# proycon/analiticcl

Measured on AMD Instinct MI355X. Metric: scored (query,candidate) pairs/sec + queries/sec, 200k-lexicon, len≤16, 1/2/4/8 GPU, higher is better.
Workload: dtype u8

## Files before the change

### analiticcl_amd/csrc/engine.hip

```cpp
#include <hip/hip_runtime.h>

#include <algorithm>
#include <atomic>
#include <functional>
#include <chrono>
#include <cmath>
#include <cstdio>
#include <cstdlib>
#include <cstring>
#include <map>
#include <memory>
#include <mutex>
#include <unordered_map>
#include <numeric>
#include <thread>
#include <type_traits>

#include "engine_internal.h"

namespace anx {

#define HIP_TRY(expr)                                                                          \
  do {                                                                                         \
    hipError_t _e = (expr);                                                                    \
// ... 1008 lines not shown
      if (hipEventElapsedTime(&ms, r.e0, r.e1) == hipSuccess) { auto& a = t.acc[r.name]; a.first += ms; a.second += 1; }
    }
    if (r.e0) (void)hipEventDestroy(r.e0);
    if (r.e1) (void)hipEventDestroy(r.e1);
  }
  t.pending.clear();
  ++t.generation;
}
}
int ktimer_begin(const char* name, hipStream_t st) {
  KTimer& t = ktimer();
  if (!t.on.load(std::memory_order_relaxed)) return -1;
  KTimerRec r;
  r.name = name;
  if (hipEventCreate(&r.e0) != hipSuccess || hipEventCreate(&r.e1) != hipSuccess || hipEventRecord(r.e0, st) != hipSuccess) {
    if (r.e0) (void)hipEventDestroy(r.e0);
    if (r.e1) (void)hipEventDestroy(r.e1);
    return -1;
  }
  std::lock_guard<std::mutex> lk(t.mu);
  if (t.pending.size() >= 0xFFFFu) return -1;
  t.pending.push_back(r);
  return (int)(((t.generation & 0x7FFFu) << 16) | (uint32_t)(t.pending.size() - 1));
}
void ktimer_end(int handle, hipStream_t st) {
  if (handle < 0) return;
  KTimer& t = ktimer();
  std::lock_guard<std::mutex> lk(t.mu);
  const uint32_t idx = (uint32_t)handle & 0xFFFFu;
  if ((((uint32_t)handle >> 16) & 0x7FFFu) != (t.generation & 0x7FFFu) || idx >= t.pending.size()) return;
  KTimerRec& r = t.pending[idx];
  if (hipEventRecord(r.e1, st) == hipSuccess) r.closed = true;
}
void kernel_timer_enable(bool on) {
  KTimer& t = ktimer();
  std::lock_guard<std::mutex> lk(t.mu);
  ktimer_resolve_locked(t);
  t.acc.clear();
  t.on.store(on);
}
bool kernel_timer_read(const char* name, double* total_ms, uint64_t* launches) {
  KTimer& t = ktimer();
  std::lock_guard<std::mutex> lk(t.mu);
  ktimer_resolve_locked(t);
  auto it = t.acc.find(name ? name : "");
  if (it == t.acc.end()) { if (total_ms) *total_ms = 0.0; if (launches) *launches = 0; return false; }
  if (total_ms) *total_ms = it->second.first;
  if (launches) *launches = it->second.second;
  return true;
}

#include "launch_plan.hpp"

template <int NP>
static void launch_scan(ScanArgs A, uint32_t nadj, uint32_t nbits, uint32_t nsad, hipStream_t st, hipEvent_t e0, hipEvent_t e1) {
  (void)hipEventRecord(e0, st);
  const bool gen = A.want_exact || A.qpairs || !A.drop_len;
  if (nadj) {
    A.ntiles = nadj;
    if (gen) hipLaunchKernelGGL((k_scan_adj<true>), dim3((nadj + 3) / 4), dim3(256), 0, st, A);
    else hipLaunchKernelGGL((k_scan_adj<false>), dim3((nadj + 3) / 4), dim3(256), 0, st, A);
    A.tiles += nadj;
    nbits -= nadj;
  }
  if (nbits) {
    A.ntiles = nbits;
    if (A.want_exact || A.qpairs || !A.drop_len) hipLaunchKernelGGL((k_scan_bits<true>), dim3((nbits + 3) / 4), dim3(256), 0, st, A);
    else hipLaunchKernelGGL((k_scan_bits<false>), dim3((nbits + 3) / 4), dim3(256), 0, st, A);
  }
  (void)hipEventRecord(e1, st);
  if (nsad) {
    A.tiles += nbits;
    A.ntiles = nsad;
    hipLaunchKernelGGL((k_scan_sad<NP>), dim3((nsad + 3) / 4), dim3(256), 0, st, A);
  }
}

static int ensure_raw(Batch* b, size_t slots_per_region, std::string& err) {
  uint32_t shift = 10;
  while (((size_t)1 << shift) < slots_per_region) ++shift;
  if (shift > 25) { err = "pair list exceeds 2^31 slots: split the batch"; return ANX_ELIMIT; }
  const size_t cap = (size_t)SCAN_REGIONS << shift;
  if (cap <= b->raw_cap) return ANX_OK;
  for (void* p : {(void*)b->raw, (void*)b->p_score, (void*)b->p_meta})
    if (p) pool_free(p);
  b->raw = nullptr; b->p_score = nullptr; b->p_meta = nullptr; b->raw_cap = 0;
  int rc;
  if ((rc = dalloc(&b->raw, cap, err))) return rc;
  b->raw_cap = cap;
  b->region_shift = shift;
  return ANX_OK;
}
static int ensure_pair_outputs(Batch* b, std::string& err) {
  if (b->p_meta) return ANX_OK;
  int rc;
  if ((rc = dalloc(&b->p_score, b->raw_cap, err)) || (rc = dalloc(&b->p_meta, b->raw_cap, err))) return rc;
  return ANX_OK;
}

static int ensure_surv(Batch* b, size_t cap, std::string& err) {
  if (cap <= b->surv_cap) return ANX_OK;
  for (void* p : {(void*)b->c_rows, (void*)b->r_rows, (void*)b->t_key})
    if (p) pool_free(p);
  b->c_rows = nullptr;
  b->r_rows = nullptr;
  b->t_key = nullptr;
  b->surv_cap = 0;
  int rc;
  if ((rc = dalloc(&b->c_rows, cap, err)) || (rc = dalloc(&b->r_rows, cap, err)) || (rc = dalloc(&b->t_key, cap, err))) return rc;
  b->surv_cap = cap;
  return ANX_OK;
}
static int ensure_surv_records(Batch* b, size_t need, std::string& err) {
  if (need <= b->surv_region_cap) return ANX_OK;
// ... 713 lines not shown
```

### analiticcl_amd/csrc/host_model.cpp

```cpp
#include "host_model.h"
#include "adjacency.h"

#include <sched.h>

#include <thread>

#include <algorithm>
#include <cmath>
#include <cstdio>
#include <cstring>
#include <fstream>
#include <numeric>
#include <sstream>

#include "unicode_tables.inc"

namespace anx {

static std::vector<uint32_t> make_primes() {
  std::vector<uint32_t> p;
  for (uint32_t n = 2; p.size() < 168; ++n) {
    bool prime = true;
    for (uint32_t d : p) {
      if (d * d > n) break;
// ... 448 lines not shown
    for (;;) {
      size_t e = line.find('\t', pos);
      fields.emplace_back(line, pos, e == std::string::npos ? std::string::npos : e - pos);
      if (e == std::string::npos) break;
      pos = e + 1;
    }
    bool havef = false;
    uint32_t freq = 0;
    if (has_freq < 0) {
      if (fields.size() >= 2 && (fields.size() - 2) % 3 == 0) {
        if (parse_u32(fields[1], freq)) { has_freq = 1; havef = true; }
      } else has_freq = 0;
    } else if (has_freq == 1) {
      if (fields.size() < 2 || !parse_u32(fields[1], freq)) {
        err = "Frequency must be an integer (line " + std::to_string(linenr) + ", column 2)";
        return ANX_EINVAL;
      }
      havef = true;
    }
    const uint64_t ref_id = add_to_vocabulary(fields[0].c_str(), havef, freq, p, lexidx);
    const size_t step = has_freq == 1 ? 3 : 2;
    for (size_t i = has_freq == 1 ? 2 : 1; i + step - 1 < fields.size(); i += step) {
      char* endp = nullptr;
      const double score = strtod(fields[i + 1].c_str(), &endp);
      if (fields[i + 1].empty() || *endp) { err = "Variant scores must be a floating point value (line " + std::to_string(linenr) + ")"; return ANX_EINVAL; }
      uint32_t vf = 0;
      if (has_freq == 1 && !parse_u32(fields[i + 2], vf)) { err = "Variant frequency must be an integer (line " + std::to_string(linenr) + ")"; return ANX_EINVAL; }
      add_variant(ref_id, fields[i].c_str(), score, has_freq == 1, vf, transparent ? tp : p, lexidx);
    }
  }
  lexicons.push_back(path);
  return ANX_OK;
}

static int pick_planes(int nsym) {
  const int need = (nsym + 3) / 4;
  for (int v : {8, 16, 24, 32, 42})
    if (need <= v) return v;
  return -1;
}

namespace {
struct SwitchDef { const char* name; void (*set)(Switches&, const char*); };
int flag01(const char* v, int dflt) { return !v ? dflt : (v[0] == '0' ? 0 : 1); }
const SwitchDef kSwitches[] = {
    {"ANX_ENCODE", [](Switches& s, const char* v) { s.encode_host = v && strcmp(v, "host") == 0; }},
    {"ANX_SCAN", [](Switches& s, const char* v) { s.scan_sad = v && strcmp(v, "sad") == 0; }},
    {"ANX_SCAN_WALK", [](Switches& s, const char* v) { s.scan_walk_flat = v && strcmp(v, "flat") == 0; }},
    {"ANX_SCAN_TQ", [](Switches& s, const char* v) { const int x = v ? atoi(v) : 0; s.scan_tq = x >= 1 && x <= 64 ? x : 0; }},
    {"ANX_SCAN_ADJ", [](Switches& s, const char* v) { s.scan_adj = flag01(v, 1); }},
    {"ANX_ADJ_BUILD", [](Switches& s, const char* v) { s.adj_build_host = v && strcmp(v, "host") == 0; }},
    {"ANX_ADJ_CLOSURE", [](Switches& s, const char* v) { const int x = v ? atoi(v) : 2; s.adj_closure = x >= 0 && x <= kAdjMaxClosure ? x : kAdjMaxClosure; }},
    {"ANX_SCAN_CHUNK_FUSED", [](Switches& s, const char* v) { const int x = v ? atoi(v) : 0; s.scan_chunk_fused = x >= 32 && x <= 1024 ? x : 0; }},
    {"ANX_ADJ_FAIL", [](Switches& s, const char* v) { s.adj_fail = flag01(v, 0); }},
    {"ANX_SMALL", [](Switches& s, const char* v) { s.small_path = flag01(v, 1); }},
    {"ANX_SURV_SEG", [](Switches& s, const char* v) { const int x = v ? atoi(v) : 32; s.surv_seg = x >= 0 && x <= 256 ? x : 32; }},
    {"ANX_ENC_PRIORITY", [](Switches& s, const char* v) { s.enc_priority = flag01(v, 1); }},
    {"ANX_HINTS", [](Switches& s, const char* v) { s.hints = flag01(v, 1); }},
    {"ANX_ADJ_MB", [](Switches& s, const char* v) { const long x = v ? atol(v) : 0; s.adj_budget_mb = x > 0 ? x : 16384; }},
    {"ANX_SIG_GROUPS", [](Switches& s, const char* v) { const int x = v ? atoi(v) : 0; s.sig_groups = x >= 1 && x <= 8 ? x : 0; }},
    {"ANX_PREFILTER", [](Switches& s, const char* v) { s.prefilter = flag01(v, 1); }},
    {"ANX_SCORE_FAST", [](Switches& s, const char* v) { s.score_fast = flag01(v, 1); }},
    {"ANX_FS_SPLIT", [](Switches& s, const char* v) { s.fs_split = flag01(v, 1); }},
    {"ANX_FS_PLANES", [](Switches& s, const char* v) { s.fs_planes = flag01(v, 1); }},
    {"ANX_FS_B7", [](Switches& s, const char* v) { s.fs_b7 = flag01(v, 1); }},
    {"ANX_SCAN_FUSE", [](Switches& s, const char* v) { s.fuse_prefilter = flag01(v, 1); }},
    {"ANX_CAP_DIV", [](Switches& s, const char* v) { const long x = v ? atol(v) : 0; s.cap_div = x > 1 ? x : 1; }},
    {"ANX_MAX_BATCH", [](Switches& s, const char* v) { const long x = v ? atol(v) : 0; s.max_batch = x > 0 ? x : (4l << 20); }},
    {"ANX_RUN_OVERLAP", [](Switches& s, const char* v) { s.run_overlap = (v && atoi(v) == 0 && v[0] == '0') ? 0 : 1; }},
    {"ANX_SHARD_POLICY", [](Switches& s, const char* v) { s.shard_by_length = (v && strcmp(v, "range") == 0) ? 0 : 1; }},
    {"ANX_SHARD_MIN", [](Switches& s, const char* v) { const long x = v ? atol(v) : 0; s.shard_min = x > 0 ? x : 8192; }},
    {"ANX_CONFUSABLES", [](Switches& s, const char* v) { s.confusables_host = v && strcmp(v, "host") == 0; }},
    {"ANX_LATTICE", [](Switches& s, const char* v) { s.lattice_host = v && strcmp(v, "host") == 0; }},
    {"ANX_SEARCH_ONEPASS", [](Switches& s, const char* v) { s.search_onepass = flag01(v, 1); }},
    {"ANX_ENCODE_TIMING", [](Switches& s, const char* v) { s.encode_timing = v != nullptr && v[0] != 0 && v[0] != '0'; }},
    {"ANX_SEARCH_TIMING", [](Switches& s, const char* v) { s.search_timing = v != nullptr && v[0] != 0 && v[0] != '0'; }},
    {"ANX_SEARCH_PARTS", [](Switches& s, const char* v) { const int x = v ? atoi(v) : 0; s.search_parts = x >= 1 && x <= 8 ? x : 4; }},
    {"ANX_SEARCH_PART_BYTES", [](Switches& s, const char* v) { const long x = v ? atol(v) : 0; s.search_part_bytes = x > 0 ? x : (4l << 20); }},
    {"ANX_SEARCH_PRIO", [](Switches& s, const char* v) { s.search_prio = flag01(v, 1); }},
    {"ANX_SEARCH_EARLY_OUTPUT", [](Switches& s, const char* v) { s.search_early_output = flag01(v, 1); }},
    {"ANX_SEARCH_FIRST_PCT", [](Switches& s, const char* v) { const int x = v ? atoi(v) : 0; s.search_first_pct = x >= 10 && x <= 100 ? x : 50; }},
    {"ANX_SEARCH_PARTS_MIN", [](Switches& s, const char* v) { const long x = v ? atol(v) : 0; s.search_parts_min = x > 0 ? x : (2l << 20); }},
    {"ANX_LEARN_FOLD", [](Switches& s, const char* v) { s.learn_fold_host = v && strcmp(v, "host") == 0; }},
    {"ANX_LEARN_HASH_BITS", [](Switches& s, const char* v) { const int x = v ? atoi(v) : 63; s.learn_hash_bits = x >= 1 && x <= 63 ? x : 63; }},
};
}
Switches& switches() {
  static Switches sw = []() {
    Switches s;
    for (const SwitchDef& d : kSwitches)
      if (const char* v = getenv(d.name)) d.set(s, v);
    return s;
  }();
  return sw;
}
bool set_switch(const char* name, const char* value) {
  if (!name) return false;
  for (const SwitchDef& d : kSwitches)
    if (strcmp(d.name, name) == 0) { d.set(switches(), value); return true; }
  return false;
}

unsigned usable_hw_threads() {
  static const unsigned cached = []() {
    unsigned n = std::max(1u, std::thread::hardware_concurrency());
    cpu_set_t set;
// ... 256 lines not shown
```

### analiticcl_amd/csrc/host_model.h

```cpp
#pragma once
#include <cstdint>
#include <atomic>
#include <memory>
#include <mutex>
#include <string>
#include <unordered_map>
#include <vector>

#include "../../include/anx.h"
#include "confusables_core.hpp"
#include "contextrules_flat.hpp"

namespace anx {

constexpr int kMaxSymbols = 255;
constexpr int kMaxAlphabet = 166;
constexpr int kMaxAnagramDistance = 12;
constexpr int kMaxEditDistance = 12;

struct AlphabetMember {
  std::string bytes;
  int nchars;
};

struct Alphabet {
  std::vector<std::vector<AlphabetMember>> classes;
  int size() const { return (int)classes.size(); }
  struct Cand { int16_t cls; const AlphabetMember* m; };
  std::vector<Cand> by_first[256];
  int16_t fast[256];
  void index();
  bool scan(const char* text, size_t nbytes, std::vector<int16_t>& out) const;
  int scan_into(const char* text, size_t nbytes, int16_t* out, int cap) const;
};

bool parse_alphabet(const std::string& tsv, Alphabet& out, std::string& err);
struct EncodeTables {
  int16_t fast[256];
  uint32_t coff[257];
  std::vector<uint32_t> cand;
  std::vector<uint8_t> bytes;
  std::vector<uint32_t> lower;
};
void build_encode_tables(const Alphabet& a, EncodeTables& out);
bool first_char_is_lowercase(const char* utf8);
bool is_alphabetic_cp(uint32_t cp);
const uint32_t (*alphabetic_ranges(uint32_t* n))[2];
uint32_t utf8_decode_at(const char* s, size_t avail, int* len);
std::string trim_whitespace(const std::string& s);
unsigned usable_hw_threads();

struct Switches {
  int encode_host = 0;
  int scan_sad = 0;
  int scan_walk_flat = 0;
  int scan_tq = 0;
  int scan_adj = 1;
  int adj_build_host = 0;
  int adj_closure = 2;
  long adj_budget_mb = 16384;
  int sig_groups = 0;
  int prefilter = 1;
  int score_fast = 1;
  int fs_planes = 1;
  int fs_split = 1;
  int fs_b7 = 1;
  int fuse_prefilter = 1;
  long cap_div = 1;
  long max_batch = 4l << 20;
  int run_overlap = 1;
  int shard_by_length = 1;
  long shard_min = 8192;
  int confusables_host = 0;
  int lattice_host = 0;
  int search_onepass = 1;
  int scan_chunk_fused = 0;
  int adj_fail = 0;
  int small_path = 1;
  int enc_priority = 1;
  int hints = 1;
  int encode_timing = 0;
  int search_timing = 0;
  int search_parts = 4;
  long search_parts_min = 2l << 20;
  long search_part_bytes = 4l << 20;
  int search_prio = 1;
  int search_early_output = 1;
  int search_first_pct = 50;
  int surv_seg = 32;
  int learn_fold_host = 0;
  int learn_hash_bits = 63;
};
Switches& switches();
bool set_switch(const char* name, const char* value);

struct VariantRef {
  bool variant_of;
  uint64_t id;
  double score;
};

struct VocabEntry {
  std::string text;
  std::vector<uint8_t> norm;
  uint32_t frequency;
  uint32_t lexindex;
  uint8_t tokencount;
  uint8_t vocabtype;
  bool has_variants = false;
  std::vector<VariantRef> variants;
};

struct BigVal {
  std::vector<uint32_t> w;
  void set_one() { w.assign(1, 1u); }
  void mul_small(uint32_t m);
  int cmp(const BigVal& o) const;
  std::string to_decimal() const;
};

struct LexiconImage {
  int nsym = 0;
  int nplanes = 0;
  uint32_t nclasses = 0, nentries = 0;
  std::vector<uint32_t> cls_planes;
  uint32_t cstride = 0;
  std::vector<uint32_t> cls_bits;
  std::vector<uint8_t> cls_len;
  std::vector<uint32_t> cls_off;
// ... 147 lines not shown
```

### analiticcl_amd/csrc/kernels_scan.hpp

```cpp
#pragma once

enum { RC_RAW = 0, RC_VALID = 1, RC_FUSED = 2 , RC_TESTS = 4 ,
       RC_ADJ = 14 , RC_ADJ_FIRST = 15  };

struct WaveOut {
  uint32_t base, left;
  uint32_t emitted;
  uint32_t nbase;
  uint32_t split;
  uint32_t rbase, rend;
  uint32_t* ctr;
  uint32_t chunk;
};
__device__ inline uint32_t wave_inclusive_scan(uint32_t x) {
  uint32_t v = x;
  v += (uint32_t)__builtin_amdgcn_update_dpp(0, (int)x, 0x111, 0xF, 0xF, false);
  v += (uint32_t)__builtin_amdgcn_update_dpp(0, (int)x, 0x112, 0xF, 0xF, false);
  v += (uint32_t)__builtin_amdgcn_update_dpp(0, (int)x, 0x113, 0xF, 0xF, false);
  v += (uint32_t)__builtin_amdgcn_update_dpp(0, (int)v, 0x114, 0xF, 0xE, false);
  v += (uint32_t)__builtin_amdgcn_update_dpp(0, (int)v, 0x118, 0xF, 0xC, false);
  v += (uint32_t)__builtin_amdgcn_update_dpp(0, (int)v, 0x142, 0xA, 0xF, false);
  v += (uint32_t)__builtin_amdgcn_update_dpp(0, (int)v, 0x143, 0xC, 0xF, false);
  return v;
}
__device__ inline uint32_t wave_reserve(WaveOut& w, uint32_t ntot, uint32_t lane, uint32_t* total_out) {
  const uint32_t incl = wave_inclusive_scan(ntot);
  const uint32_t total = (uint32_t)__builtin_amdgcn_readlane((int)incl, 63);
  *total_out = total;
  w.split = w.left;
  if (total > w.left) {
    const uint32_t rest = total - w.left;
    const uint32_t need = rest > w.chunk ? rest : w.chunk;
    uint32_t b = 0;
    if (lane == 0) b = atomicAdd(&w.ctr[RC_RAW], need);
    w.nbase = w.rbase + __shfl(b, 0);
  }
  return incl - ntot;
}
__device__ inline void wave_reserve_total(WaveOut& w, uint32_t total, uint32_t lane) {
  w.split = w.left;
  if (total > w.left) {
    const uint32_t rest = total - w.left;
    const uint32_t need = rest > w.chunk ? rest : w.chunk;
    uint32_t b = 0;
    if (lane == 0) b = atomicAdd(&w.ctr[RC_RAW], need);
    w.nbase = w.rbase + (uint32_t)__builtin_amdgcn_readfirstlane((int)b);
  }
}
__device__ inline uint32_t wave_slot(const WaveOut& w, uint32_t g) {
  return g < w.split ? w.base + g : w.nbase + (g - w.split);
}
__device__ inline void wave_commit(WaveOut& w, uint32_t total) {
  if (total > w.left) {
    const uint32_t rest = total - w.left;
    const uint32_t need = rest > w.chunk ? rest : w.chunk;
    w.base = w.nbase + rest;
    w.left = need - rest;
  } else {
    w.base += total;
    w.left -= total;
  }
  w.emitted += total;
}
__device__ inline void wave_close(const WaveOut& w, uint32_t lane, uint2* __restrict__ raw) {
  for (uint32_t i = lane; i < w.left; i += 64)
    if (w.base + i < w.rend) raw[w.base + i] = make_uint2(RAW_INVALID, 0u);
  if (lane == 0 && w.emitted) atomicAdd(&w.ctr[RC_VALID], w.emitted);
}

struct ScanArgs {
  const Tile* tiles;
  uint32_t ntiles;
  const uint32_t* q_bits;
  const uint32_t* q_cv;
  const uint32_t* cls_bits;
  const uint32_t* cls_planes;
  const uint4* scan_rec;
  const uint2* scan_rec34;
  uint32_t pad_rec;
  uint32_t cstride;
  uint32_t pad_class;
  const uint8_t* cls_len;
  const uint32_t* cls_off;
  const uint4* sig;
  const uint4* sig_e;
  const uint4* sighash;
  const uint4* sighash_e;
  uint32_t hash_mask;
  const unsigned long long* ball;
  const uint32_t* adj_hdr;
  const uint2* adj_planes;
  const uint32_t* adj_ids;
  const uint32_t* sig_cbeg;
  uint2* raw;
  uint32_t region_cap;
  uint32_t chunk;
  uint32_t chunk_fused;
  uint32_t* rctr;
  const uint32_t* qexact;
  int want_exact;
  int drop_len;
  const uint4* q_rec;
  const uint4* e_rec;
  int fuse;
  uint32_t* qpairs;
  int dbg;
};

__device__ inline int32_t bcnt_acc(uint32_t x, int32_t acc) {
  int32_t r;
  asm("v_bcnt_u32_b32 %0, %1, %2" : "=v"(r) : "v"(x), "v"(acc));
  return r;
}
__device__ inline int32_t bcnt_acc_s(uint32_t x, int32_t acc) {
  int32_t r;
  asm("v_bcnt_u32_b32 %0, %1, %2" : "=v"(r) : "v"(x), "s"(acc));
  return r;
}

template <bool BITS, int NP, bool GEN, bool ADJ = false>
__device__ inline void scan_tile(const ScanArgs& AA, const Tile& t, uint32_t item, uint32_t* __restrict__ stage, uint32_t* __restrict__ hits,
                                 uint32_t* __restrict__ qlds, uint4* __restrict__ qsym, uint32_t* __restrict__ pbuf) {
  ScanArgs A = AA;
  if (!GEN) { A.want_exact = 0; A.qpairs = nullptr; A.drop_len = 1; A.qexact = nullptr; }
  constexpr int CPL = BITS ? 4 : (NP <= 8 ? 4 : NP <= 16 ? 2 : 1);
  constexpr int W = BITS ? NBITPLANES : NP;
  constexpr int QSTRIDE = BITS ? NBITPLANES : NP;
  constexpr uint32_t CHUNK = 64u * CPL;
  const uint32_t lane = threadIdx.x & 63;
  const uint32_t* __restrict__ cls_words = BITS ? A.cls_bits : A.cls_planes;
  const uint8_t* __restrict__ cls_len = A.cls_len;
  const uint32_t* __restrict__ cls_off = A.cls_off;
  uint2* __restrict__ raw = A.raw;
  const uint32_t cstride = A.cstride;
  const uint32_t region = item % SCAN_REGIONS;
  WaveOut wo{0, 0, 0, 0, 0, region * A.region_cap, (region + 1) * A.region_cap, A.rctr + region * RC_STRIDE, A.chunk};
  uint32_t ns = 0;
  uint32_t nchunks = 0;
  uint32_t arend = 0;
  int32_t alc[4] = {0, 0, 0, 0};
  uint2 apl[4] = {};
  uint32_t aid[4] = {};
  auto adj_load = [&](uint32_t row, uint2 (&pl)[4], uint32_t (&id)[4]) {
#pragma unroll
    for (int j = 0; j < 4; ++j) {
      pl[j] = make_uint2(0u, 0u);
      id[j] = A.pad_rec;
      if (row + (uint32_t)j < arend) {
        const size_t p = (size_t)(row + (uint32_t)j) * 64u + lane;
        pl[j] = A.adj_planes[p];
        id[j] = A.adj_ids[p];
      }
    }
  };
  {
    const uint32_t* __restrict__ src = (BITS ? A.q_bits : A.q_cv) + (size_t)t.q0 * QSTRIDE;
    for (uint32_t i = lane; i < t.nq * QSTRIDE; i += 64) qlds[i] = src[i];
  }
  const bool fuse = BITS && A.fuse && t.lq <= 16u && t.d <= 3u;
  if (fuse) wo.chunk = A.chunk_fused;
  if (BITS && fuse && lane < t.nq) qsym[lane] = rec32(A.q_rec, t.q0 + lane)[0];
  constexpr uint32_t PBUF = SCAN_PBUF;
  uint32_t nfused = 0;
  uint32_t npb = 0, phead = 0;

  uint32_t nhits = 0;
  uint32_t counted_only = 0;
  auto emit_dense = [&](bool fin) {
    while (npb >= 64u || (fin && npb)) {
      const uint32_t cnt = npb < 64u ? npb : 64u;
      const bool act = lane < cnt;
      const uint32_t pr = pbuf[(phead + lane) & (PBUF - 1u)];
      const uint32_t e = act ? (pr & 0x3FFFFFFu) : 0u, ql = act ? (pr >> 26) : 0u;
      bool keep = act;
      uint32_t flag = 0u;
      if (ANX_DBG(A.dbg) & 16) keep = false;
      if (BITS && fuse && !(ANX_DBG(A.dbg) & 16)) {
        nfused += cnt;
        const uint4 C = rec32(A.e_rec, e)[0];
        const int lc = (int)(rec32(A.e_rec, e)[1].x & 0xFFu), lq = (int)t.lq, d = (int)t.d;
        const uint4 Q = qsym[ql];
        const bool filt = act && lc <= 16;
        const int ml = lq > lc ? lq : lc;
        constexpr uint32_t M = 0x7F7F7F7Fu;
        bool rej;
        if (__any(filt && ml > 12)) {
          const uint32_t q4[4] = {Q.x & M, Q.y & M, Q.z & M, Q.w & M}, c6[6] = {M, C.x & M, C.y & M, C.z & M, C.w & M, M};
          rej = band_bound_rejects<4, true, true>(q4, c6, filt, d, lq, lc);
        } else if (__any(filt && ml > 8)) {
          const uint32_t q3[3] = {Q.x & M, Q.y & M, Q.z & M}, c5[5] = {M, C.x & M, C.y & M, C.z & M, M};
          rej = band_bound_rejects<3, true, true>(q3, c5, filt, d, lq, lc);
        } else {
          const uint32_t q2[2] = {Q.x & M, Q.y & M}, c4[4] = {M, C.x & M, C.y & M, M};
          rej = band_bound_rejects<2, true, true>(q2, c4, filt, d, lq, lc);
        }
        if (rej) { keep = false; ++counted_only; }
        if (filt) flag = RAW_PREFILTERED;
      }
      if (ANX_DBG(A.dbg) & 32) keep = false;
      const unsigned long long km = __ballot(keep);
      const uint32_t total = (uint32_t)__popcll(km);
      if (total) {
        wave_reserve_total(wo, total, lane);
        if (keep) {
          const uint32_t q = t.q0 + ql;
          uint32_t exact = 0u;
          if (A.want_exact) exact = A.qexact[q] == A.scan_rec[e].w ? 0x80000000u : 0u;
          const uint32_t g = __builtin_amdgcn_mbcnt_hi((uint32_t)(km >> 32), __builtin_amdgcn_mbcnt_lo((uint32_t)km, 0u));
          const uint32_t pos = wave_slot(wo, g);
          if (pos < wo.rend) raw[pos] = make_uint2(q, e | exact | flag);
        }
        wave_commit(wo, total);
      }
      phead = (phead + cnt) & (PBUF - 1u);
      npb -= cnt;
    }
  };
  auto flush = [&]() {
    for (uint32_t r0 = 0; r0 < nhits; r0 += 64) {
      const uint32_t idx = r0 + lane;
      uint32_t c = 0, m = 0, e0 = 0, ne = 0, qb = 0;
      if (idx < nhits) {
        bool count_only;
        if (BITS) {
          const uint32_t hx = reinterpret_cast<const uint16_t*>(hits + SCAN_HITS)[idx];
          m = hits[idx];
          qb = ((hx >> 8) & 1u) << 5;
          count_only = (hx >> 9) & 1u;
          e0 = stage[hx & 0xFFu];
          ne = 1;
          c = A.qpairs ? A.scan_rec[e0].w : 0u;
        } else {
          c = hits[2 * idx];
          m = hits[2 * idx + 1];
          qb = ((c >> 27) & 1u) << 5;
          c &= (1u << 27) - 1u;
          const uint32_t lc = cls_len[c];
          e0 = cls_off[c];
          ne = cls_off[c + 1] - e0;
          const uint32_t diff = lc > t.lq ? lc - t.lq : t.lq - lc;
          count_only = A.drop_len && diff > t.d;
        }
        if (A.qpairs) {
          for (uint32_t mm = m; mm; mm &= mm - 1u) {
            const uint32_t q = t.q0 + qb + (uint32_t)__ffs((int)mm) - 1u;
            if (!A.want_exact || A.qexact[q] == 0xFFFFFFFFu || A.qexact[q] == c) atomicAdd(&A.qpairs[q], ne);
          }
        }
        if (count_only) {
          counted_only += (uint32_t)__popc(m) * ne;
          m = 0;
        }
      }
      if (BITS) {
        while (true) {
          const bool has = m != 0u;
          const unsigned long long bm = __ballot(has);
          if (!bm) break;
          if (has) {
            const uint32_t bit = (uint32_t)__ffs((int)m) - 1u;
            m &= m - 1u;
            pbuf[(phead + npb + __builtin_amdgcn_mbcnt_hi((uint32_t)(bm >> 32), __builtin_amdgcn_mbcnt_lo((uint32_t)bm, 0u))) & (PBUF - 1u)] = e0 | ((qb + bit) << 26);
          }
          npb += (uint32_t)__popcll(bm);
          if (npb >= 64u) emit_dense(false);
// ... 151 lines not shown
      if (!BITS && nhits > SCAN_HITS - CHUNK) flush();
    }
    if (BITS) flush();
  };

  uint32_t* __restrict__ sdelta = stage + CHUNK;
  uint32_t* __restrict__ smask = stage + CHUNK + 64;
  auto stage_runs = [&](bool ok, uint32_t cb, uint32_t n) {
    ok = ok && n != 0u;
    const unsigned long long okm = __ballot(ok);
    if (!okm || (ANX_DBG(A.dbg) & 4)) return;
    const uint32_t cnt = ok ? n : 0u;
    const uint32_t incl = wave_inclusive_scan(cnt);
    const uint32_t carry = ns & 63u;
    const uint32_t total = carry + (uint32_t)__builtin_amdgcn_readlane((int)incl, 63);
    uint32_t wbase = ns - carry;
    const uint32_t endp = carry + incl - 1u;
    if (ok) sdelta[__builtin_amdgcn_mbcnt_hi((uint32_t)(okm >> 32), __builtin_amdgcn_mbcnt_lo((uint32_t)okm, 0u))] = cb + cnt - 1u - endp;
    uint32_t rbase = 0;
    for (uint32_t w0 = 0; w0 < total; w0 += SCAN_MASKW) {
      if (lane < SCAN_MASKW / 32u) smask[lane] = 0u;
      if (ok && endp - w0 < SCAN_MASKW) atomicOr(smask + ((endp - w0) >> 5), 1u << (endp & 31u));
      const uint32_t wend = total < w0 + SCAN_MASKW ? total : w0 + SCAN_MASKW;
      for (uint32_t p0 = w0; p0 < wend; p0 += 64) {
        const uint32_t mlo = (uint32_t)__builtin_amdgcn_readfirstlane((int)smask[((p0 - w0) >> 6) * 2u]), mhi = (uint32_t)__builtin_amdgcn_readfirstlane((int)smask[((p0 - w0) >> 6) * 2u + 1u]);
        const uint32_t r = rbase + __builtin_amdgcn_mbcnt_hi(mhi, __builtin_amdgcn_mbcnt_lo(mlo, 0u));
        rbase += (uint32_t)__popc(mlo) + (uint32_t)__popc(mhi);
        const uint32_t p = p0 + lane;
        const uint32_t id = sdelta[r & 63u] + p;
        if (p >= carry && p < total) stage[wbase + lane] = id;
        if (p0 + 64u <= total) {
          wbase += 64u;
          ns = wbase;
          if (wbase == CHUNK) {
            process();
            ns = 0;
            wbase = 0;
          }
        } else {
          ns = wbase + (total - p0);
        }
      }
    }
  };
  const uint4* __restrict__ sigtab = BITS ? A.sig_e : A.sig;
  if (ADJ) {
    const cptr_u32 hp = (cptr_u32)(A.adj_hdr + (size_t)(t.adj - 1u) * 8u);
    const uint32_t row0 = hp[0], c0 = hp[1], c1 = hp[2], c2 = hp[3], c3 = hp[4], c4 = hp[5], c5 = hp[6], c6 = hp[7];
    uint32_t rbeg = t.k >= 3u ? 0u : t.k == 2u ? c0 : t.k == 1u ? c1 : c2;
    uint32_t rend = t.k >= 3u ? c6 : t.k == 2u ? c5 : t.k == 1u ? c4 : c3;
    if (t.flags & 2u) { rbeg = t.s0; rend = t.s1; }
    arend = row0 + rend;
    if (lane == 0 && rend > rbeg) {
      atomicAdd(&wo.ctr[RC_ADJ], rend - rbeg);
      if (t.flags & 1u) atomicAdd(&wo.ctr[RC_ADJ_FIRST], rend - rbeg);
    }
    uint2 npl[4];
    uint32_t nid[4];
    if (rbeg < rend) adj_load(row0 + rbeg, npl, nid);
    for (uint32_t r = rbeg; r < rend; r += (uint32_t)CPL) {
#pragma unroll
      for (int j = 0; j < 4; ++j) {
        const uint32_t rr = r + (uint32_t)j;
        alc[j] = (int32_t)t.lq - 3 + (int32_t)((rr >= c0) + (rr >= c1) + (rr >= c2) + (rr >= c3) + (rr >= c4) + (rr >= c5));
        apl[j] = npl[j];
        aid[j] = nid[j];
      }
      if (r + (uint32_t)CPL < rend) adj_load(row0 + r + (uint32_t)CPL, npl, nid);
      process();
    }
  } else if (t.balln) {
    const unsigned long long H = 0x8080808080808080ull;
    const unsigned long long sq = (unsigned long long)t.sig_lo | (unsigned long long)t.sig_hi << 32;
    const uint4* __restrict__ htab = BITS ? A.sighash_e : A.sighash;
    for (uint32_t base = 0; base < t.balln; base += 64) {
      const uint32_t i = base + lane;
      bool found = false;
      uint32_t first = 0, count = 0;
      if (i < t.balln) {
        const unsigned long long dl = A.ball[t.ball0 + i];
        const unsigned long long r = ((sq & ~H) + (dl & ~H)) ^ ((sq ^ dl) & H);
        if (!(r & (r << 1) & H)) {
          const uint32_t lo = (uint32_t)r, hi = (uint32_t)(r >> 32);
          uint32_t h = sig_hash(lo, hi) & A.hash_mask;
          for (int p = 0; p < 17; ++p) {
            const uint4 e = htab[h];
            if (!e.w) break;
            if (e.x == lo && e.y == hi) { found = true; first = e.z; count = e.w; break; }
            h = (h + 1u) & A.hash_mask;
          }
        }
      }
      stage_runs(found, first, count);
    }
  } else {
    const uint4* __restrict__ sigp = sigtab + t.s0 + lane;
    uint4 sg_next = t.s0 < t.s1 ? *sigp : make_uint4(0xFFFFFFFFu, 0xFFFFFFFFu, 0u, 0u);
    for (uint32_t sb = t.s0; sb < t.s1; sb += 64) {
      const uint4 sg = sg_next;
      sigp += 64;
      if (sb + 64 < t.s1) sg_next = *sigp;
      const bool ok = __builtin_amdgcn_sad_u8(sg.x, t.sig_lo, __builtin_amdgcn_sad_u8(sg.y, t.sig_hi, 0u)) <= t.k;
      stage_runs(ok, sg.z, sg.w);
    }
  }
  if (!ADJ && ns) process();
  flush();
  if (BITS) emit_dense(true);
  if (A.drop_len) {
    const uint32_t tot = (uint32_t)__builtin_amdgcn_readlane((int)wave_inclusive_scan(counted_only), 63);
    wo.emitted += tot;
  }
  wave_close(wo, lane, raw);
  if (BITS && lane == 0 && nfused) atomicAdd(&wo.ctr[RC_FUSED], nfused);
  if (lane == 0 && nchunks) {
    if (BITS) {
      const uint32_t e[5] = {0u, t.kend & 0xFFu, (t.kend >> 8) & 0xFFu, (t.kend >> 16) & 0xFFu, t.nq};
      for (int k = 1; k <= NBITPLANES; ++k)
        if (e[k] > e[k - 1])
          atomicAdd(reinterpret_cast<unsigned long long*>(wo.ctr + RC_TESTS + 2 * k), (unsigned long long)nchunks * CHUNK * (e[k] - e[k - 1]));
    } else {
      atomicAdd(reinterpret_cast<unsigned long long*>(wo.ctr + RC_TESTS), (unsigned long long)nchunks * CHUNK * t.nq);
    }
  }
}

constexpr uint32_t SCAN_STAGE = 64 * 4 + 64 + SCAN_MASKW / 32;
template <int NP, bool BITS, bool GEN, bool ADJ = false>
__device__ inline void scan_wave(const ScanArgs& A) {
  constexpr int QWORDS = SCAN_TQ * (BITS ? NBITPLANES : NP);
  __shared__ uint32_t s_qlds[4][QWORDS];
  __shared__ __attribute__((aligned(16))) uint32_t s_stage[4][ADJ ? 64 * 4 : SCAN_STAGE];
  __shared__ uint32_t s_hits[4][BITS ? SCAN_HITS + SCAN_HITS / 2 : 2 * SCAN_HITS];
  __shared__ uint4 s_qsym[BITS ? 4 : 1][BITS ? SCAN_TQ : 1];
  __shared__ uint32_t s_pbuf[BITS ? 4 : 1][BITS ? SCAN_PBUF : 1];
  const uint32_t wid = threadIdx.x >> 6;
  const uint32_t item = (uint32_t)__builtin_amdgcn_readfirstlane((int)(blockIdx.x * 4u + wid));
  if (item >= A.ntiles) return;
  const cptr_u32 tp = (cptr_u32)(A.tiles + item);
  Tile t;
  t.q0 = tp[0]; t.nq = tp[1]; t.s0 = tp[2]; t.s1 = tp[3]; t.k = tp[4]; t.lq = tp[5]; t.sig_lo = tp[6]; t.sig_hi = tp[7]; t.kind = tp[8]; t.d = tp[9]; t.kend = tp[10]; t.ball0 = tp[11]; t.balln = tp[12]; t.adj = tp[13]; t.flags = tp[14];
  scan_tile<BITS, NP, GEN, ADJ>(A, t, item, s_stage[wid], s_hits[wid], s_qlds[wid], s_qsym[BITS ? wid : 0], s_pbuf[BITS ? wid : 0]);
}
template <bool GEN>
__global__ __launch_bounds__(256) __attribute__((amdgpu_waves_per_eu(5, 8))) void k_scan_bits(ScanArgs A) { scan_wave<8, true, GEN>(A); }
template <bool GEN>
__global__ __launch_bounds__(256) __attribute__((amdgpu_waves_per_eu(6, 8))) void k_scan_adj(ScanArgs A) { scan_wave<8, true, GEN, true>(A); }
template <int NP>
__global__ __launch_bounds__(256) void k_scan_sad(ScanArgs A) { scan_wave<NP, false, true>(A); }


template <int NP>
__global__ __launch_bounds__(256) void k_scan_small(ScanArgs A) {
  constexpr int QW = NP > NBITPLANES ? NP : NBITPLANES;
  __shared__ uint32_t s_qlds[4][QW];
  __shared__ __attribute__((aligned(16))) uint32_t s_stage[4][SCAN_STAGE];
  __shared__ uint32_t s_hits[4][2 * SCAN_HITS];
  __shared__ uint4 s_qsym[4][1];
  __shared__ uint32_t s_pbuf[4][SCAN_PBUF];
  const uint32_t wid = threadIdx.x >> 6;
  const uint32_t item = (uint32_t)__builtin_amdgcn_readfirstlane((int)(blockIdx.x * 4u + wid));
  if (item >= A.ntiles) return;
  const cptr_u32 tp = (cptr_u32)(A.tiles + item);
  Tile t;
  t.q0 = tp[0]; t.nq = tp[1]; t.s0 = tp[2]; t.s1 = tp[3]; t.k = tp[4]; t.lq = tp[5]; t.sig_lo = tp[6]; t.sig_hi = tp[7]; t.kind = tp[8]; t.d = tp[9]; t.kend = tp[10]; t.ball0 = tp[11]; t.balln = tp[12]; t.adj = tp[13]; t.flags = tp[14];
  if (t.nq == 0u) return;
  if (t.kind == 0u) scan_tile<false, NP, true>(A, t, item, s_stage[wid], s_hits[wid], s_qlds[wid], s_qsym[wid], s_pbuf[wid]);
  else if (t.adj) scan_tile<true, 8, false, true>(A, t, item, s_stage[wid], s_hits[wid], s_qlds[wid], s_qsym[wid], s_pbuf[wid]);
  else scan_tile<true, 8, false>(A, t, item, s_stage[wid], s_hits[wid], s_qlds[wid], s_qsym[wid], s_pbuf[wid]);
}
```

Before: 54.71 billion.

## Add persistent ticket-based tile scheduling for adjacency scan kernel

Adds an optional persistent-kernel mode for the adjacency scan. Waves grab tiles from eight striped atomic ticket counters instead of one tile per wave, and the grid is capped at the resident block count from an occupancy query. Per-tile counter atomics are replaced by per-wave LDS accumulators that are flushed once at the end or on overflow. The mode is gated behind ANX_SCAN_TICKET and is off by default. The default path still uses the restructured kernel with LDS stat accumulation and kernarg-pointer reloads, which may change register usage.

```diff
diff --git a/analiticcl_amd/csrc/engine.hip b/analiticcl_amd/csrc/engine.hip
--- a/analiticcl_amd/csrc/engine.hip
+++ b/analiticcl_amd/csrc/engine.hip
@@ -1084,14 +1084,38 @@
 
 #include "launch_plan.hpp"
 
+template <bool GEN>
+static uint32_t scan_adj_resident_blocks() {
+  constexpr int kMaxDev = 64;
+  static std::mutex mu;
+  static uint32_t cached[kMaxDev] = {};
+  int dev = 0;
+  if (hipGetDevice(&dev) != hipSuccess || dev < 0 || dev >= kMaxDev) dev = 0;
+  std::lock_guard<std::mutex> g(mu);
+  if (!cached[dev]) {
+    int per_cu = 0, cus = 0;
+    if (hipOccupancyMaxActiveBlocksPerMultiprocessor(&per_cu, k_scan_adj<GEN>, 256, 0) != hipSuccess) per_cu = 0;
+    if (hipDeviceGetAttribute(&cus, hipDeviceAttributeMultiprocessorCount, dev) != hipSuccess) cus = 0;
+    (void)hipGetLastError();
+    cached[dev] = per_cu > 0 && cus > 0 ? (uint32_t)per_cu * (uint32_t)cus : 1536u;
+  }
+  return cached[dev];
+}
+
 template <int NP>
 static void launch_scan(ScanArgs A, uint32_t nadj, uint32_t nbits, uint32_t nsad, hipStream_t st, hipEvent_t e0, hipEvent_t e1) {
   (void)hipEventRecord(e0, st);
   const bool gen = A.want_exact || A.qpairs || !A.drop_len;
   if (nadj) {
     A.ntiles = nadj;
-    if (gen) hipLaunchKernelGGL((k_scan_adj<true>), dim3((nadj + 3) / 4), dim3(256), 0, st, A);
-    else hipLaunchKernelGGL((k_scan_adj<false>), dim3((nadj + 3) / 4), dim3(256), 0, st, A);
+    uint32_t blocks = (nadj + 3) / 4;
+    A.ticket = switches().scan_ticket ? 1 : 0;
+    if (A.ticket) {
+      blocks = std::min(blocks, gen ? scan_adj_resident_blocks<true>() : scan_adj_resident_blocks<false>());
+      if (switches().scan_waves) blocks = std::min(blocks, (uint32_t)switches().scan_waves);
+    }
+    if (gen) hipLaunchKernelGGL((k_scan_adj<true>), dim3(blocks), dim3(256), 0, st, A);
+    else hipLaunchKernelGGL((k_scan_adj<false>), dim3(blocks), dim3(256), 0, st, A);
     A.tiles += nadj;
     nbits -= nadj;
   }
diff --git a/analiticcl_amd/csrc/host_model.cpp b/analiticcl_amd/csrc/host_model.cpp
--- a/analiticcl_amd/csrc/host_model.cpp
+++ b/analiticcl_amd/csrc/host_model.cpp
@@ -524,6 +524,8 @@
     {"ANX_ADJ_BUILD", [](Switches& s, const char* v) { s.adj_build_host = v && strcmp(v, "host") == 0; }},
     {"ANX_ADJ_CLOSURE", [](Switches& s, const char* v) { const int x = v ? atoi(v) : 2; s.adj_closure = x >= 0 && x <= kAdjMaxClosure ? x : kAdjMaxClosure; }},
     {"ANX_SCAN_CHUNK_FUSED", [](Switches& s, const char* v) { const int x = v ? atoi(v) : 0; s.scan_chunk_fused = x >= 32 && x <= 1024 ? x : 0; }},
+    {"ANX_SCAN_TICKET", [](Switches& s, const char* v) { s.scan_ticket = flag01(v, 0); }},
+    {"ANX_SCAN_WAVES", [](Switches& s, const char* v) { const int x = v ? atoi(v) : 0; s.scan_waves = x >= 1 ? x : 0; }},
     {"ANX_ADJ_FAIL", [](Switches& s, const char* v) { s.adj_fail = flag01(v, 0); }},
     {"ANX_SMALL", [](Switches& s, const char* v) { s.small_path = flag01(v, 1); }},
     {"ANX_SURV_SEG", [](Switches& s, const char* v) { const int x = v ? atoi(v) : 32; s.surv_seg = x >= 0 && x <= 256 ? x : 32; }},
diff --git a/analiticcl_amd/csrc/host_model.h b/analiticcl_amd/csrc/host_model.h
--- a/analiticcl_amd/csrc/host_model.h
+++ b/analiticcl_amd/csrc/host_model.h
@@ -75,6 +75,8 @@
   int lattice_host = 0;
   int search_onepass = 1;
   int scan_chunk_fused = 0;
+  int scan_ticket = 0;
+  int scan_waves = 0;
   int adj_fail = 0;
   int small_path = 1;
   int enc_priority = 1;
diff --git a/analiticcl_amd/csrc/kernels_scan.hpp b/analiticcl_amd/csrc/kernels_scan.hpp
--- a/analiticcl_amd/csrc/kernels_scan.hpp
+++ b/analiticcl_amd/csrc/kernels_scan.hpp
@@ -1,7 +1,10 @@
 #pragma once
 
 enum { RC_RAW = 0, RC_VALID = 1, RC_FUSED = 2 , RC_TESTS = 4 ,
-       RC_ADJ = 14 , RC_ADJ_FIRST = 15  };
+       RC_ADJ = 14 , RC_ADJ_FIRST = 15 ,
+       RC_TICKET = 16  };
+constexpr uint32_t SCAN_TICKETS = 8;
+enum { WS_ADJ = 0, WS_ADJ_FIRST = 1, WS_FUSED = 2, WS_VALID = 3 , WS_TESTS = 3 , WS_N = 8 };
 
 struct WaveOut {
   uint32_t base, left;
@@ -50,7 +53,7 @@
 __device__ inline uint32_t wave_slot(const WaveOut& w, uint32_t g) {
   return g < w.split ? w.base + g : w.nbase + (g - w.split);
 }
-__device__ inline void wave_commit(WaveOut& w, uint32_t total) {
+__device__ inline void wave_commit(WaveOut& w, uint32_t total, uint32_t* stat = nullptr, uint32_t lane = 0) {
   if (total > w.left) {
     const uint32_t rest = total - w.left;
     const uint32_t need = rest > w.chunk ? rest : w.chunk;
@@ -60,7 +63,11 @@
     w.base += total;
     w.left -= total;
   }
-  w.emitted += total;
+  if (stat) {
+    if (lane == 0) stat[WS_VALID] += total;
+  } else {
+    w.emitted += total;
+  }
 }
 __device__ inline void wave_close(const WaveOut& w, uint32_t lane, uint2* __restrict__ raw) {
   for (uint32_t i = lane; i < w.left; i += 64)
@@ -102,6 +109,7 @@
   int drop_len;
   const uint4* q_rec;
   const uint4* e_rec;
+  int ticket;
   int fuse;
   uint32_t* qpairs;
   int dbg;
@@ -118,8 +126,8 @@
   return r;
 }
 
-template <bool BITS, int NP, bool GEN, bool ADJ = false>
-__device__ inline void scan_tile(const ScanArgs& AA, const Tile& t, uint32_t item, uint32_t* __restrict__ stage, uint32_t* __restrict__ hits,
+template <bool BITS, int NP, bool GEN, bool ADJ = false, bool WSTAT = false>
+__device__ inline void scan_tile(const ScanArgs& AA, const Tile& t, WaveOut& wo, uint32_t* __restrict__ stat, uint32_t* __restrict__ stage, uint32_t* __restrict__ hits,
                                  uint32_t* __restrict__ qlds, uint4* __restrict__ qsym, uint32_t* __restrict__ pbuf) {
   ScanArgs A = AA;
   if (!GEN) { A.want_exact = 0; A.qpairs = nullptr; A.drop_len = 1; A.qexact = nullptr; }
@@ -133,8 +141,6 @@
   const uint32_t* __restrict__ cls_off = A.cls_off;
   uint2* __restrict__ raw = A.raw;
   const uint32_t cstride = A.cstride;
-  const uint32_t region = item % SCAN_REGIONS;
-  WaveOut wo{0, 0, 0, 0, 0, region * A.region_cap, (region + 1) * A.region_cap, A.rctr + region * RC_STRIDE, A.chunk};
   uint32_t ns = 0;
   uint32_t nchunks = 0;
   uint32_t arend = 0;
@@ -158,7 +164,7 @@
     for (uint32_t i = lane; i < t.nq * QSTRIDE; i += 64) qlds[i] = src[i];
   }
   const bool fuse = BITS && A.fuse && t.lq <= 16u && t.d <= 3u;
-  if (fuse) wo.chunk = A.chunk_fused;
+  wo.chunk = fuse ? A.chunk_fused : A.chunk;
   if (BITS && fuse && lane < t.nq) qsym[lane] = rec32(A.q_rec, t.q0 + lane)[0];
   constexpr uint32_t PBUF = SCAN_PBUF;
   uint32_t nfused = 0;
@@ -176,7 +182,8 @@
       uint32_t flag = 0u;
       if (ANX_DBG(A.dbg) & 16) keep = false;
       if (BITS && fuse && !(ANX_DBG(A.dbg) & 16)) {
-        nfused += cnt;
+        if (WSTAT) { if (lane == 0) stat[WS_FUSED] += cnt; }
+        else nfused += cnt;
         const uint4 C = rec32(A.e_rec, e)[0];
         const int lc = (int)(rec32(A.e_rec, e)[1].x & 0xFFu), lq = (int)t.lq, d = (int)t.d;
         const uint4 Q = qsym[ql];
@@ -210,7 +217,7 @@
           const uint32_t pos = wave_slot(wo, g);
           if (pos < wo.rend) raw[pos] = make_uint2(q, e | exact | flag);
         }
-        wave_commit(wo, total);
+        wave_commit(wo, total, WSTAT ? stat : nullptr, lane);
       }
       phead = (phead + cnt) & (PBUF - 1u);
       npb -= cnt;
@@ -468,8 +475,13 @@
     if (t.flags & 2u) { rbeg = t.s0; rend = t.s1; }
     arend = row0 + rend;
     if (lane == 0 && rend > rbeg) {
-      atomicAdd(&wo.ctr[RC_ADJ], rend - rbeg);
-      if (t.flags & 1u) atomicAdd(&wo.ctr[RC_ADJ_FIRST], rend - rbeg);
+      if (WSTAT) {
+        stat[WS_ADJ] += rend - rbeg;
+        if (t.flags & 1u) stat[WS_ADJ_FIRST] += rend - rbeg;
+      } else {
+        atomicAdd(&wo.ctr[RC_ADJ], rend - rbeg);
+        if (t.flags & 1u) atomicAdd(&wo.ctr[RC_ADJ_FIRST], rend - rbeg);
+      }
     }
     uint2 npl[4];
     uint32_t nid[4];
@@ -525,43 +537,128 @@
   if (BITS) emit_dense(true);
   if (A.drop_len) {
     const uint32_t tot = (uint32_t)__builtin_amdgcn_readlane((int)wave_inclusive_scan(counted_only), 63);
-    wo.emitted += tot;
-  }
-  wave_close(wo, lane, raw);
-  if (BITS && lane == 0 && nfused) atomicAdd(&wo.ctr[RC_FUSED], nfused);
+    if (!WSTAT) wo.emitted += tot;
+    else if (lane == 0) stat[WS_VALID] += tot;
+  }
+  if (BITS && !WSTAT && lane == 0 && nfused) atomicAdd(&wo.ctr[RC_FUSED], nfused);
   if (lane == 0 && nchunks) {
     if (BITS) {
       const uint32_t e[5] = {0u, t.kend & 0xFFu, (t.kend >> 8) & 0xFFu, (t.kend >> 16) & 0xFFu, t.nq};
       for (int k = 1; k <= NBITPLANES; ++k)
-        if (e[k] > e[k - 1])
-          atomicAdd(reinterpret_cast<unsigned long long*>(wo.ctr + RC_TESTS + 2 * k), (unsigned long long)nchunks * CHUNK * (e[k] - e[k - 1]));
+        if (e[k] > e[k - 1]) {
+          if (WSTAT) stat[WS_TESTS + k] += nchunks * (e[k] - e[k - 1]);
+          else atomicAdd(reinterpret_cast<unsigned long long*>(wo.ctr + RC_TESTS + 2 * k), (unsigned long long)nchunks * CHUNK * (e[k] - e[k - 1]));
+        }
     } else {
       atomicAdd(reinterpret_cast<unsigned long long*>(wo.ctr + RC_TESTS), (unsigned long long)nchunks * CHUNK * t.nq);
     }
   }
 }
+__device__ inline WaveOut wave_open(const ScanArgs& A, uint32_t region) {
+  return WaveOut{0, 0, 0, 0, 0, region * A.region_cap, (region + 1) * A.region_cap, A.rctr + region * RC_STRIDE, A.chunk};
+}
+template <bool BITS, int NP, bool GEN, bool ADJ = false>
+__device__ inline void scan_one_tile(const ScanArgs& A, const Tile& t, uint32_t item, uint32_t* __restrict__ stage, uint32_t* __restrict__ hits,
+                                     uint32_t* __restrict__ qlds, uint4* __restrict__ qsym, uint32_t* __restrict__ pbuf) {
+  WaveOut wo = wave_open(A, item % SCAN_REGIONS);
+  scan_tile<BITS, NP, GEN, ADJ, false>(A, t, wo, nullptr, stage, hits, qlds, qsym, pbuf);
+  wave_close(wo, threadIdx.x & 63, A.raw);
+}
+__device__ inline Tile load_tile(const Tile* tiles, uint32_t item) {
+  const cptr_u32 tp = (cptr_u32)(tiles + item);
+  Tile t;
+  t.q0 = tp[0]; t.nq = tp[1]; t.s0 = tp[2]; t.s1 = tp[3]; t.k = tp[4]; t.lq = tp[5]; t.sig_lo = tp[6]; t.sig_hi = tp[7]; t.kind = tp[8]; t.d = tp[9]; t.kend = tp[10]; t.ball0 = tp[11]; t.balln = tp[12]; t.adj = tp[13]; t.flags = tp[14];
+  return t;
+}
 
 constexpr uint32_t SCAN_STAGE = 64 * 4 + 64 + SCAN_MASKW / 32;
-template <int NP, bool BITS, bool GEN, bool ADJ = false>
+template <int NP, bool BITS, bool GEN>
 __device__ inline void scan_wave(const ScanArgs& A) {
   constexpr int QWORDS = SCAN_TQ * (BITS ? NBITPLANES : NP);
   __shared__ uint32_t s_qlds[4][QWORDS];
-  __shared__ __attribute__((aligned(16))) uint32_t s_stage[4][ADJ ? 64 * 4 : SCAN_STAGE];
+  __shared__ __attribute__((aligned(16))) uint32_t s_stage[4][SCAN_STAGE];
   __shared__ uint32_t s_hits[4][BITS ? SCAN_HITS + SCAN_HITS / 2 : 2 * SCAN_HITS];
   __shared__ uint4 s_qsym[BITS ? 4 : 1][BITS ? SCAN_TQ : 1];
   __shared__ uint32_t s_pbuf[BITS ? 4 : 1][BITS ? SCAN_PBUF : 1];
   const uint32_t wid = threadIdx.x >> 6;
   const uint32_t item = (uint32_t)__builtin_amdgcn_readfirstlane((int)(blockIdx.x * 4u + wid));
   if (item >= A.ntiles) return;
-  const cptr_u32 tp = (cptr_u32)(A.tiles + item);
-  Tile t;
-  t.q0 = tp[0]; t.nq = tp[1]; t.s0 = tp[2]; t.s1 = tp[3]; t.k = tp[4]; t.lq = tp[5]; t.sig_lo = tp[6]; t.sig_hi = tp[7]; t.kind = tp[8]; t.d = tp[9]; t.kend = tp[10]; t.ball0 = tp[11]; t.balln = tp[12]; t.adj = tp[13]; t.flags = tp[14];
-  scan_tile<BITS, NP, GEN, ADJ>(A, t, item, s_stage[wid], s_hits[wid], s_qlds[wid], s_qsym[BITS ? wid : 0], s_pbuf[BITS ? wid : 0]);
+  const Tile t = load_tile(A.tiles, item);
+  scan_one_tile<BITS, NP, GEN>(A, t, item, s_stage[wid], s_hits[wid], s_qlds[wid], s_qsym[BITS ? wid : 0], s_pbuf[BITS ? wid : 0]);
+}
+
+__device__ inline void stats_flush(uint32_t* ctr, uint32_t* stat) {
+  if (stat[WS_ADJ]) atomicAdd(&ctr[RC_ADJ], stat[WS_ADJ]);
+  if (stat[WS_ADJ_FIRST]) atomicAdd(&ctr[RC_ADJ_FIRST], stat[WS_ADJ_FIRST]);
+  if (stat[WS_FUSED]) atomicAdd(&ctr[RC_FUSED], stat[WS_FUSED]);
+  if (stat[WS_VALID]) atomicAdd(&ctr[RC_VALID], stat[WS_VALID]);
+  for (int k = 1; k <= NBITPLANES; ++k)
+    if (stat[WS_TESTS + k]) atomicAdd(reinterpret_cast<unsigned long long*>(ctr + RC_TESTS + 2 * k), (unsigned long long)stat[WS_TESTS + k] * 256u);
+  for (int i = 0; i < WS_N; ++i) stat[i] = 0u;
+}
+template <bool GEN>
+__device__ inline void scan_wave_adj(const ScanArgs& A) {
+  __shared__ uint32_t s_qlds[4][SCAN_TQ * NBITPLANES];
+  __shared__ __attribute__((aligned(16))) uint32_t s_stage[4][64 * 4];
+  __shared__ uint32_t s_hits[4][SCAN_HITS + SCAN_HITS / 2];
+  __shared__ uint4 s_qsym[4][SCAN_TQ];
+  __shared__ uint32_t s_pbuf[4][SCAN_PBUF];
+  enum { WL_WORD = WS_N, WL_LEFT = WS_N + 1, WL_ARGS = WS_N + 2 , WL_N = WS_N + 4 };
+  __shared__ uint32_t s_wave[4][WL_N];
+  const uint32_t wid = threadIdx.x >> 6, lane = threadIdx.x & 63;
+  uint32_t* __restrict__ stat = s_wave[wid];
+  auto bcast = [](uint32_t x) { return (uint32_t)__builtin_amdgcn_readfirstlane((int)x); };
+  (void)A;
+  if (lane == 0) {
+    const unsigned long long ka = (unsigned long long)__builtin_amdgcn_kernarg_segment_ptr();
+    stat[WL_ARGS] = (uint32_t)ka;
+    stat[WL_ARGS + 1] = (uint32_t)(ka >> 32);
+  }
+  auto kargs = [&]() {
+    return (const __attribute__((address_space(4))) ScanArgs*)((unsigned long long)bcast(stat[WL_ARGS]) | (unsigned long long)bcast(stat[WL_ARGS + 1]) << 32);
+  };
+  const uint32_t gw = bcast(blockIdx.x * 4u + wid);
+  WaveOut wo = wave_open(*(const ScanArgs*)kargs(), gw % SCAN_REGIONS);
+  if (lane == 0) {
+    for (int i = 0; i < WS_N; ++i) stat[i] = 0u;
+    stat[WL_WORD] = gw % SCAN_TICKETS;
+    stat[WL_LEFT] = SCAN_TICKETS;
+  }
+  auto request = [&](uint32_t tw) {
+    uint32_t v = 0;
+    if (lane == 0) v = atomicAdd(kargs()->rctr + tw * RC_STRIDE + RC_TICKET, 1u);
+    return v;
+  };
+  auto tile_of = [&](uint32_t v, uint32_t ntiles) {
+    uint32_t tw = bcast(stat[WL_WORD]);
+    uint32_t it = bcast(v) * SCAN_TICKETS + tw;
+    if (it >= ntiles) {
+      uint32_t left = bcast(stat[WL_LEFT]);
+      while (it >= ntiles && --left) {
+        tw = (tw + 1u) % SCAN_TICKETS;
+        it = bcast(request(tw)) * SCAN_TICKETS + tw;
+      }
+      if (lane == 0) { stat[WL_WORD] = tw; stat[WL_LEFT] = left; }
+    }
+    return it;
+  };
+  uint32_t item = kargs()->ticket ? tile_of(request(gw % SCAN_TICKETS), kargs()->ntiles) : gw;
+  while (item < kargs()->ntiles) {
+    const Tile t = load_tile(kargs()->tiles, item);
+    uint32_t next = 0;
+    if (kargs()->ticket) next = request(bcast(stat[WL_WORD]));
+    scan_tile<true, 8, GEN, true, true>(*(const ScanArgs*)kargs(), t, wo, stat, s_stage[wid], s_hits[wid], s_qlds[wid], s_qsym[wid], s_pbuf[wid]);
+    if (!kargs()->ticket) break;
+    if (lane == 0 && ((stat[WS_TESTS + 1] | stat[WS_TESTS + 2] | stat[WS_TESTS + 3] | stat[WS_TESTS + 4] | stat[WS_FUSED] | stat[WS_VALID] | stat[WS_ADJ]) >> 30)) stats_flush(wo.ctr, stat);
+    item = tile_of(next, kargs()->ntiles);
+  }
+  wave_close(wo, lane, kargs()->raw);
+  if (lane == 0) stats_flush(wo.ctr, stat);
 }
 template <bool GEN>
 __global__ __launch_bounds__(256) __attribute__((amdgpu_waves_per_eu(5, 8))) void k_scan_bits(ScanArgs A) { scan_wave<8, true, GEN>(A); }
 template <bool GEN>
-__global__ __launch_bounds__(256) __attribute__((amdgpu_waves_per_eu(6, 8))) void k_scan_adj(ScanArgs A) { scan_wave<8, true, GEN, true>(A); }
+__global__ __launch_bounds__(256) __attribute__((amdgpu_waves_per_eu(6, 8))) void k_scan_adj(ScanArgs A) { scan_wave_adj<GEN>(A); }
 template <int NP>
 __global__ __launch_bounds__(256) void k_scan_sad(ScanArgs A) { scan_wave<NP, false, true>(A); }
 
@@ -577,11 +674,9 @@
   const uint32_t wid = threadIdx.x >> 6;
   const uint32_t item = (uint32_t)__builtin_amdgcn_readfirstlane((int)(blockIdx.x * 4u + wid));
   if (item >= A.ntiles) return;
-  const cptr_u32 tp = (cptr_u32)(A.tiles + item);
-  Tile t;
-  t.q0 = tp[0]; t.nq = tp[1]; t.s0 = tp[2]; t.s1 = tp[3]; t.k = tp[4]; t.lq = tp[5]; t.sig_lo = tp[6]; t.sig_hi = tp[7]; t.kind = tp[8]; t.d = tp[9]; t.kend = tp[10]; t.ball0 = tp[11]; t.balln = tp[12]; t.adj = tp[13]; t.flags = tp[14];
+  const Tile t = load_tile(A.tiles, item);
   if (t.nq == 0u) return;
-  if (t.kind == 0u) scan_tile<false, NP, true>(A, t, item, s_stage[wid], s_hits[wid], s_qlds[wid], s_qsym[wid], s_pbuf[wid]);
-  else if (t.adj) scan_tile<true, 8, false, true>(A, t, item, s_stage[wid], s_hits[wid], s_qlds[wid], s_qsym[wid], s_pbuf[wid]);
-  else scan_tile<true, 8, false>(A, t, item, s_stage[wid], s_hits[wid], s_qlds[wid], s_qsym[wid], s_pbuf[wid]);
-}
+  if (t.kind == 0u) scan_one_tile<false, NP, true>(A, t, item, s_stage[wid], s_hits[wid], s_qlds[wid], s_qsym[wid], s_pbuf[wid]);
+  else if (t.adj) scan_one_tile<true, 8, false, true>(A, t, item, s_stage[wid], s_hits[wid], s_qlds[wid], s_qsym[wid], s_pbuf[wid]);
+  else scan_one_tile<true, 8, false>(A, t, item, s_stage[wid], s_hits[wid], s_qlds[wid], s_qsym[wid], s_pbuf[wid]);
+}
```

After: 53.36 billion. -2.5%, worse.
